# lightonai/next-plaid

Measured on AMD Instinct MI355X. Metric: queries/sec + p50 latency, k=10, 10M-doc x 300-tok x d128 PLAID index, 1/2/4/8 GPU, higher is better.
Workload: dtype f32 (split-bf16 hi/lo MFMA on the residual term of MaxSim, f32-class accuracy)

## Files before the change

next-plaid_amd/csrc/np_kernels.h:

```cpp
#pragma once
#include <hip/hip_runtime.h>
#include <stdint.h>
#include "np_exact.h"

namespace np {

__device__ __forceinline__ int wave_max_nonneg(int v) {
  v = max(v, __builtin_amdgcn_update_dpp(0, v, 0x111, 0xf, 0xf, false));
  v = max(v, __builtin_amdgcn_update_dpp(0, v, 0x112, 0xf, 0xf, false));
  v = max(v, __builtin_amdgcn_update_dpp(0, v, 0x114, 0xf, 0xf, false));
  v = max(v, __builtin_amdgcn_update_dpp(0, v, 0x118, 0xf, 0xf, false));
  v = max(v, __builtin_amdgcn_update_dpp(0, v, 0x142, 0xa, 0xf, false));
  v = max(v, __builtin_amdgcn_update_dpp(0, v, 0x143, 0xc, 0xf, false));
  return __builtin_amdgcn_readlane(v, 63);
}
template <int G, int J>
__device__ __forceinline__ int group_lane(int v, int lane) {
  if constexpr (G == 2) return __builtin_amdgcn_mov_dpp(v, J == 0 ? 0xA0 : 0xF5, 0xf, 0xf, true);
  else if constexpr (G == 4) return __builtin_amdgcn_mov_dpp(v, J == 0 ? 0x00 : 0x55, 0xf, 0xf, true);
  else return __shfl(v, (lane & ~(G - 1)) + J);
}

struct Counters {
  unsigned long long n_cells, n_ivf_ids, n_candidates, n_cand_tokens, n_exact_docs, n_exact_tokens, n_cand_codes;
// ... 982 lines not shown
    const uint32_t total = s_items[1024];
    for (uint32_t it = (uint32_t)wave; it < total; it += 16) {
      int a = 0, z = m;
      while (z - a > 1) {
        const int mid = (a + z) >> 1;
        if (s_items[mid] <= it) a = mid;
        else z = mid;
      }
      const uint32_t off = (it - s_items[a]) << 9, ln = s_len[a];
      const uint32_t* src = ivf + s_start[a] + off;
      uint32_t d[8];
#pragma unroll
      for (int k = 0; k < 8; ++k) {
        const uint32_t j = k * 64 + lane;
        d[k] = (off + j < ln) ? src[j] : 0xFFFFFFFFu;
      }
#pragma unroll
      for (int k = 0; k < 8; ++k) {
        const uint32_t rel = d[k] - lo;
        if (d[k] != 0xFFFFFFFFu && rel < span) {
          const uint32_t bit = 1u << (d[k] & 31);
          if (subset_bits && !(subset_bits[d[k] >> 5] & bit)) continue;
          atomicOr(&s_bits[rel >> 5], bit);
        }
      }
    }
  }
  __syncthreads();
  uint32_t* bits = docbits + (int64_t)b * NW + w0;
  for (int ch = wave; ch < slice_chunks; ch += 16) {
    const int64_t gch = (int64_t)sl * slice_chunks + ch;
    if (gch >= nchunks) break;
    int cnt = 0;
#pragma unroll
    for (int k = 0; k < NP_CHUNK_WORDS / 64; ++k) {
      const int w = ch * NP_CHUNK_WORDS + k * 64 + lane;
      if (w < nw) {
        const uint32_t v = s_bits[w];
        bits[w] = v;
        cnt += __popc(v);
      }
    }
#pragma unroll
    for (int o = 32; o > 0; o >>= 1) cnt += __shfl_xor(cnt, o);
    if (lane == 0) chunk_counts[(int64_t)b * nchunks + gch] = cnt;
  }
  if (sl == 0) {
#pragma unroll
    for (int o = 32; o > 0; o >>= 1) ids += __shfl_xor(ids, o);
    if (lane == 0 && ids) atomicAdd(&ctr->n_ivf_ids, ids);
  }
}

__global__ void __launch_bounds__(256) count_chunks_kernel(const uint32_t* __restrict__ docbits, int64_t NW,
                                                           int nchunks, int32_t* __restrict__ chunk_counts) {
  __shared__ int s_cnt;
  const int b = blockIdx.y, ch = blockIdx.x;
  if (threadIdx.x == 0) s_cnt = 0;
  __syncthreads();
  const uint32_t* bits = docbits + (int64_t)b * NW;
  int c = 0;
  for (int k = 0; k < NP_CHUNK_WORDS / 256; ++k) {
    const int64_t w = (int64_t)ch * NP_CHUNK_WORDS + k * 256 + threadIdx.x;
    if (w < NW) c += __popc(bits[w]);
  }
#pragma unroll
  for (int o = 32; o > 0; o >>= 1) c += __shfl_xor(c, o);
  if ((threadIdx.x & 63) == 0) atomicAdd(&s_cnt, c);
  __syncthreads();
  if (threadIdx.x == 0) chunk_counts[(int64_t)b * nchunks + ch] = s_cnt;
}

struct RoundPlan {
  int32_t* n_cand;
  int64_t* cand_base;
  int32_t* round_of;
  int32_t* round_tab;
  int32_t* order;
};

__global__ void __launch_bounds__(256) plan_rounds_kernel(const int32_t* __restrict__ chunk_counts, int nchunks, int B,
                                                          int64_t pool, int max_rounds, RoundPlan rp, Counters* ctr,
                                                          const int32_t* __restrict__ n_direct = nullptr ) {
  __shared__ int s_n[256];
  const int tid = threadIdx.x, lane = tid & 63, wave = tid >> 6;
  for (int b = wave; b < B; b += 4) {
    int c = 0;
    if (n_direct) c = lane == 0 ? n_direct[b] : 0;
    else
    for (int j = lane; j < nchunks; j += 64) c += chunk_counts[(int64_t)b * nchunks + j];
#pragma unroll
    for (int o = 32; o > 0; o >>= 1) c += __shfl_xor(c, o);
    if (lane == 0) s_n[b] = c;
  }
  __syncthreads();
  if (tid == 0) {
    int64_t cur = 0;
    unsigned long long total = 0;
    int r = 0;
    for (int i = 0; i < 2 * max_rounds; ++i) rp.round_tab[i] = 0;
    rp.round_tab[0] = 0;
    for (int b = 0; b < B; ++b) {
      const int n = s_n[b];
      if (cur + n > pool && r + 1 < max_rounds) {
        rp.round_tab[2 * r + 1] = b;
        ++r;
        rp.round_tab[2 * r] = b;
        cur = 0;
      }
      rp.n_cand[b] = (cur + n > pool) ? (int)max((int64_t)0, pool - cur) : n;
      rp.cand_base[b] = cur;
      rp.round_of[b] = r;
      cur += rp.n_cand[b];
      total += (unsigned long long)rp.n_cand[b];
    }
    rp.round_tab[2 * r + 1] = B;
    rp.round_tab[2 * max_rounds] = r + 1;
    if (!n_direct) atomicAdd(&ctr->n_candidates, total);
    atomicMax(&ctr->n_rounds, (unsigned long long)(r + 1));
  }
  __syncthreads();
  for (int b = tid; b < B; b += 256) {
    const int r = rp.round_of[b], rb = rp.round_tab[2 * r], re = rp.round_tab[2 * r + 1];
    const int n = rp.n_cand[b];
    int rank = 0;
    for (int j = rb; j < re; ++j) {
      const int nj = rp.n_cand[j];
      rank += (nj > n || (nj == n && j < b)) ? 1 : 0;
    }
    rp.order[rb + rank] = b;
  }
}

template <class Steal>
__device__ __forceinline__ int xcd_next_query(int32_t* slots, int32_t* ticket, int x, int step, int B,
                                              const int32_t* order, int rb, int re, Steal&& steal) {
  if (step > B) return -3;
  int32_t* slot = slots + (int64_t)x * (B + 1) + step;
  int v = __hip_atomic_load(slot, __ATOMIC_RELAXED, __HIP_MEMORY_SCOPE_AGENT);
  if (v == -1 && atomicCAS(slot, -1, -2) == -1) {
    const int t = atomicAdd(ticket, 1) + 1;
    v = (t < re - rb) ? order[rb + t] : steal();
    __hip_atomic_store(slot, v, __ATOMIC_RELAXED, __HIP_MEMORY_SCOPE_AGENT);
    return v;
  }
  while (v == -1 || v == -2) {
    __builtin_amdgcn_s_sleep(4);
    v = __hip_atomic_load(slot, __ATOMIC_RELAXED, __HIP_MEMORY_SCOPE_AGENT);
  }
  return v;
}

__global__ void __launch_bounds__(256) compact_kernel(const uint32_t* __restrict__ docbits, int64_t NW, int nchunks,
                                                      const int32_t* __restrict__ chunk_counts,
                                                      uint32_t* __restrict__ cand, RoundPlan rp, int round,
                                                      const uint4* __restrict__ doc_meta, uint4* __restrict__ cand_meta) {
  __shared__ int s_wave[4];
  __shared__ int s_base;
  const int b = blockIdx.y, ch = blockIdx.x, tid = threadIdx.x, lane = tid & 63, wave = tid >> 6;
  if (rp.round_of[b] != round) return;
  const int32_t* cc = chunk_counts + (int64_t)b * nchunks;
  {
    int part = 0;
    for (int j = tid; j < ch; j += 256) part += cc[j];
#pragma unroll
    for (int o = 32; o > 0; o >>= 1) part += __shfl_xor(part, o);
    if (lane == 0) s_wave[wave] = part;
    __syncthreads();
    if (tid == 0) s_base = s_wave[0] + s_wave[1] + s_wave[2] + s_wave[3];
    __syncthreads();
  }
  const int base = s_base;
  __syncthreads();
  const uint32_t* bits = docbits + (int64_t)b * NW;
  const int64_t w0 = (int64_t)ch * NP_CHUNK_WORDS + tid * 4;
  uint32_t w[4];
  int cnt = 0;
#pragma unroll
  for (int k = 0; k < 4; ++k) {
    w[k] = (w0 + k < NW) ? bits[w0 + k] : 0u;
    cnt += __popc(w[k]);
  }
  int incl = cnt;
#pragma unroll
  for (int o = 1; o < 64; o <<= 1) {
    int v = __shfl_up(incl, o);
    if (lane >= o) incl += v;
  }
  if (lane == 63) s_wave[wave] = incl;
  __syncthreads();
  int woff = 0;
  for (int k = 0; k < wave; ++k) woff += s_wave[k];
  int pos = base + woff + incl - cnt;
  const int limit = rp.n_cand[b];
  uint32_t* out = cand ? cand + rp.cand_base[b] : nullptr;
  uint4* outm = cand_meta + rp.cand_base[b];
#pragma unroll
  for (int k = 0; k < 4; ++k) {
    uint32_t m = w[k];
    while (m) {
      const int bit = __ffs(m) - 1;
      m &= m - 1;
      const uint32_t d = (uint32_t)((w0 + k) * 32 + bit);
      if (pos < limit) {
        if (doc_meta) outm[pos] = doc_meta[d];
        if (out) out[pos] = d;
      }
      ++pos;
    }
  }
}

#define NP_UB_BINS 2048
#define NP_GAIN_RANGE NP_IVF_SPLIT_RANGE
// ... 1324 lines not shown
      const uint32_t sum_lo = (uint32_t)max(slo, 0);
      if (valid && jl == 0) {
        U[pbase + i] = (uint16_t)sum;
        if (hb) atomicAdd(&s_hist[min(sum_lo >> hshift, (uint32_t)(NP_UB_BINS - 1))], 1u);
      }
      __builtin_amdgcn_wave_barrier();
    }
    __syncthreads();
    if (hb)
      for (int i = tid; i < NP_UB_BINS; i += 256) {
        const uint32_t v = s_hist[i];
        if (v) atomicAdd(&hb[i], v);
      }
  }
#pragma unroll
  for (int o = 32; o > 0; o >>= 1) {
    toks += __shfl_xor(toks, o);
    ucnt += __shfl_xor(ucnt, o);
    ndoc += __shfl_xor(ndoc, o);
  }
  __shared__ unsigned long long s_cnt[3];
  __syncthreads();
  if (tid == 0) s_cnt[0] = s_cnt[1] = s_cnt[2] = 0;
  __syncthreads();
  if (lane == 0 && toks) {
    atomicAdd(&s_cnt[0], toks);
    atomicAdd(&s_cnt[1], ucnt);
    atomicAdd(&s_cnt[2], ndoc);
  }
  __syncthreads();
  if (tid == 0 && s_cnt[0] && ctr) {
    if (count_tokens) {
      atomicAdd(&ctr->n_cand_tokens, s_cnt[0]);
      atomicAdd(&ctr->n_cand_dcodes, s_cnt[1]);
    } else {
      atomicAdd(&ctr->n_level2, s_cnt[2]);
    }
    atomicAdd(&ctr->n_cand_codes, s_cnt[1]);
  }
}

__global__ void __launch_bounds__(256) ub_thr_kernel(const uint32_t* __restrict__ hist, int hshift, int slack, int n_sel,
                                                     const int32_t* __restrict__ n_cand, RoundPlan rp, int round,
                                                     const uint32_t* __restrict__ qflag, uint32_t* __restrict__ thr) {
  __shared__ uint32_t s_part[256];
  constexpr int BPT = NP_UB_BINS / 256;
  const int b = blockIdx.x, tid = threadIdx.x;
  if (rp.round_of[b] != round) return;
  if (qflag[b] != 0 || n_cand[b] <= n_sel) {
    if (tid == 0) thr[b] = 0;
    return;
  }
  const uint32_t* hb = hist + (int64_t)b * NP_UB_BINS;
  const int top = (255 - tid) * BPT;
  uint32_t mine = 0;
#pragma unroll
  for (int k4 = 0; k4 < BPT / 4; ++k4) {
    const uint4 v = *reinterpret_cast<const uint4*>(hb + top + 4 * k4);
    mine += v.x + v.y + v.z + v.w;
  }
  s_part[tid] = mine;
  __syncthreads();
  if (tid == 0) {
    uint32_t cum = 0;
    int t = 0;
    for (; t < 255; ++t) {
      if (cum + s_part[t] >= (uint32_t)n_sel) break;
      cum += s_part[t];
    }
    int bin = (255 - t) * BPT + BPT - 1;
    for (; bin > (255 - t) * BPT; --bin) {
      if (cum + hb[bin] >= (uint32_t)n_sel) break;
      cum += hb[bin];
    }
    thr[b] = (uint32_t)max(0, bin - ((slack + (1 << hshift) - 1) >> hshift));
  }
}

struct CutP {
  const uint4* src;
  const int32_t* n_src_a;
  const int32_t* n_src_b;
  const uint16_t* U;
  const uint32_t* lo;
  const uint32_t* hi;
  int zero_mode;
  const uint4* all_src;
  const int32_t* n_all;
  uint4* dst;
  const int32_t* dst_begin;
  int32_t* n_dst;
  int hshift;
  Counters* ctr;
};

__global__ void __launch_bounds__(256) ub_cut_kernel(CutP p, RoundPlan rp, int round) {
  __shared__ int s_wcnt[4], s_base;
  __shared__ unsigned long long s_cnt[2];
  const int b = blockIdx.y, tid = threadIdx.x, lane = tid & 63, wave = tid >> 6;
  if (rp.round_of[b] != round) return;
  const uint32_t lo = p.lo[b], hi = p.hi ? p.hi[b] : 0xFFFFFFFFu;
  const bool all = lo == 0;
  if (all && p.zero_mode == 1) return;
  const uint4* src = all ? p.all_src : p.src;
  const int64_t n = all ? (int64_t)p.n_all[b] : (int64_t)p.n_src_a[b] + (p.n_src_b ? p.n_src_b[b] : 0);
  const int64_t pbase = rp.cand_base[b];
  const int64_t dbase = pbase + (p.dst_begin ? p.dst_begin[b] : 0);
  if (tid == 0) s_cnt[0] = s_cnt[1] = 0;
  unsigned long long toks = 0, ucnt = 0;
  constexpr int PT = 8;
  for (int64_t i0 = (int64_t)blockIdx.x * (256 * PT); i0 < n; i0 += (int64_t)gridDim.x * (256 * PT)) {
    bool keep[PT];
    unsigned long long bal[PT];
    int wtot = 0;
#pragma unroll
    for (int k = 0; k < PT; ++k) {
      const int64_t i = i0 + k * 256 + tid;
      bool kp = i < n;
      if (kp && !all) {
        const uint32_t bin = min((uint32_t)p.U[pbase + i] >> p.hshift, (uint32_t)(NP_UB_BINS - 1));
        kp = bin >= lo && bin < hi;
      }
      keep[k] = kp;
      bal[k] = __ballot(kp);
      wtot += (int)__popcll(bal[k]);
    }
    if (lane == 0) s_wcnt[wave] = wtot;
    __syncthreads();
    if (tid == 0) {
      const int tot = s_wcnt[0] + s_wcnt[1] + s_wcnt[2] + s_wcnt[3];
      s_base = tot ? atomicAdd(&p.n_dst[b], tot) : 0;
    }
    __syncthreads();
    int pos = s_base;
    for (int k = 0; k < wave; ++k) pos += s_wcnt[k];
#pragma unroll
    for (int k = 0; k < PT; ++k) {
      if (keep[k]) {
        const uint4 m = src[pbase + i0 + k * 256 + tid];
        p.dst[dbase + pos + (int)__popcll(bal[k] & ((1ull << lane) - 1ull))] = m;
        if (all) {
          toks += (unsigned long long)(m.w >> 8);
          ucnt += (unsigned long long)m.y;
        }
      }
      pos += (int)__popcll(bal[k]);
    }
    __syncthreads();
  }
  if (all && p.ctr) {
#pragma unroll
    for (int o = 32; o > 0; o >>= 1) {
      toks += __shfl_xor(toks, o);
      ucnt += __shfl_xor(ucnt, o);
    }
    if (lane == 0 && toks) {
      atomicAdd(&s_cnt[0], toks);
      atomicAdd(&s_cnt[1], ucnt);
    }
    __syncthreads();
    if (tid == 0 && s_cnt[0]) {
      atomicAdd(&p.ctr->n_cand_tokens, s_cnt[0]);
      atomicAdd(&p.ctr->n_cand_dcodes, s_cnt[1]);
      atomicAdd(&p.ctr->n_cand_codes, s_cnt[1]);
    }
  }
}

__global__ void __launch_bounds__(256) hot_prep_kernel(const uint8_t* __restrict__ QCU, int64_t K, int64_t KP, int RB,
                                                       uint8_t* __restrict__ cmaxu ,
                                                       uint32_t* __restrict__ chist ) {
  __shared__ uint32_t s_h[256];
  const int b = blockIdx.y, tid = threadIdx.x;
  s_h[tid] = 0;
  __syncthreads();
  for (int64_t c = (int64_t)blockIdx.x * 256 + tid; c < KP; c += (int64_t)gridDim.x * 256) {
    const uint4* row = reinterpret_cast<const uint4*>(QCU + ((int64_t)b * KP + c) * RB);
    uint32_t m = 0;
    for (int j = 0; j < RB / 16; ++j) {
      const uint4 v = row[j];
      const uint32_t w4[4] = {v.x, v.y, v.z, v.w};
#pragma unroll
      for (int e = 0; e < 4; ++e)
#pragma unroll
        for (int k = 0; k < 4; ++k) m = max(m, (w4[e] >> (8 * k)) & 0xFFu);
    }
    cmaxu[(int64_t)b * KP + c] = (uint8_t)m;
    if (c < K) atomicAdd(&s_h[m], 1u);
  }
  __syncthreads();
  if (s_h[tid]) atomicAdd(&chist[(int64_t)b * 256 + tid], s_h[tid]);
}

__global__ void __launch_bounds__(256) hot_lam_kernel(const uint32_t* __restrict__ chist, int64_t K, int hot_permille,
                                                      uint32_t* __restrict__ lam) {
  __shared__ uint32_t s_h[256];
  __shared__ uint32_t s_wsum[4];
  __shared__ int s_ok;
  const int b = blockIdx.x, v = threadIdx.x, lane = v & 63, wave = v >> 6;
  if (v == 0) s_ok = 0;
  uint32_t suf = chist[(int64_t)b * 256 + v];
#pragma unroll
  for (int o = 1; o < 64; o <<= 1) {
// ... 2350 lines not shown
```

next-plaid_amd/csrc/np_search.hip:

```cpp
#include "np_internal.h"
#include "np_kernels.h"

#include <algorithm>
#include <array>
#include <cmath>
#include <stdlib.h>
#include <string.h>
#include <type_traits>
#include <utility>

namespace np {

struct Workspace {
  DevBuf q, qoff, Qt, Qb, Qbl, QCT, gmax, tauq, cellbits, cells_tmp, cells, n_cells, docbits, chunk_counts, cand, cand_meta, approx, n_cand,
      cand_base, round_of, round_tab, QCU, qinv, qflag, ub, ub_hist, ub_thr, ub_cursor, q_order, xcd_slots, surv_meta, n_surv, n_list2, sel_keys, sel_doc, nsel, exact, out_ids, out_scores, out_keys, out_counts, ctr, subset,
      subset_bits, elig, misc, cut, cmaxu, chist, ub2, ub_hist2, ub_thr2, list_meta, n_l1, n_l2, qpad, planes, levels, hotbits,
      gain, gsmall, ghist, s0_meta, s0_u, gacc, gdeep,
      scan,
      filt, filt_csr;
  void* h_pin = nullptr;
  size_t h_pin_cap = 0;
  unsigned long long* h_gain = nullptr;
  uint64_t h_gain_key = 0;
  hipEvent_t done = nullptr;
// ... 1070 lines not shown
    hot_levels_kernel<<<dim3((unsigned)std::min<int64_t>(std::max<int64_t>((KP >> 5) / 256, 1), 16), B), 256, 0, st>>>(
        w.chist.as<uint32_t>(), ix->K, ix->tune.s4_hot, w.cmaxu.as<uint8_t>(), KP, ix->tune.s4_pexp, w.ub_thr2.as<uint32_t>() + B,
        w.levels.as<uint32_t>(), w.hotbits.as<uint32_t>(), p.s4_warm, w.ub_thr2.as<uint32_t>() + 2 * B,
        w.hotbits.as<uint32_t>() + (size_t)B * (KP / 32), ix->tune.s4_hot_auto ? w.n_cand.as<int32_t>() : nullptr,
        ix->tune.s4_hot_auto);
    const dim3 pg((unsigned)std::min<int64_t>((KP + 2047) / 2048, 64), B);
    with_int<32, 64>(p.RB, [&](auto RB) {
      hot_planes_kernel<RB><<<pg, 256, 0, st>>>(w.QCU.as<uint8_t>(), KP, w.cmaxu.as<uint8_t>(), w.ub_thr2.as<uint32_t>() + B,
                                                w.levels.as<uint32_t>(), w.planes.as<uint32_t>());
    });
  }
  return NP_OK;
}

int Pass::rounds(const RoundPlan& rp, const GainP& gp) const {
  SelectP sp;
  sp.approx = w.approx.as<float>();
  sp.cand = w.cand.as<uint32_t>();
  sp.cand_step = 1;
  sp.rp = rp;
  sp.n_cand = w.n_cand.as<int32_t>();
  sp.doc_begin = ix->doc_begin;
  sp.n_sel = cs->n_sel;
  sp.NSELP = cs->NSELP;
  sp.sel_keys = w.sel_keys.as<uint64_t>();
  sp.sel_doc = w.sel_doc.as<uint32_t>();
  sp.nsel_out = w.nsel.as<int32_t>();
  sp.ctr = nullptr;
  const size_t sel_lds = (size_t)cs->NSELP * 8;
  if (cs->n_sel > 0 && sel_lds > 48 * 1024)
    NP_HIP(hipFuncSetAttribute(reinterpret_cast<const void*>(&select_kernel),
                               hipFuncAttributeMaxDynamicSharedMemorySize, (int)sel_lds));
  for (int r = 0; r < (p.have_cands ? p.max_rounds : 0); ++r) NP_TRY(round(r, rp, gp, sp));
  return NP_OK;
}

int Pass::round(int r, const RoundPlan& rp, const GainP& gp, SelectP sp) const {
  const int B = p.B;
  if (p.gain_path)
    gain_emit_kernel<2><<<dim3((unsigned)ix->n_ranges, (unsigned)B), 256, 0, st>>>(gp, r);
  else
    compact_kernel<<<dim3(p.nchunks, B), 256, 0, st>>>(w.docbits.as<uint32_t>(), p.NW, p.nchunks, w.chunk_counts.as<int32_t>(),
                                                       (p.use_filter && !p.ids_only) ? nullptr : w.cand.as<uint32_t>(), rp, r,
                                                       p.ids_only ? nullptr : ix->d_doc_meta.get(), w.cand_meta.as<uint4>());
  if (cs->timed && r == 0) NP_HIP(hipEventRecord(cs->ctx->ev[3], st));
  const bool matvec = p.batched && !p.s1_split;
  if (p.use_filter) {
    NP_TRY(p.two_level ? two_level_cut(r, rp) : single_level_cut(r, rp));
    launch_approx(st, ix, w, d_qoff, B, p.LQP, w.surv_meta.as<uint4>(), w.n_surv.as<int32_t>(), rp, r, p.max_rounds, nullptr);
    sp.cand = reinterpret_cast<const uint32_t*>(w.surv_meta.p);
    sp.cand_step = 4;
    sp.n_cand = w.n_surv.as<int32_t>();
    sp.ctr = w.ctr.as<Counters>();
    if (matvec) {
      gcut_kernel<<<B, 1024, 0, st>>>(w.approx.as<float>(), w.surv_meta.as<uint4>(), w.n_surv.as<int32_t>(), rp, r, cs->n_sel,
                                      w.qinv.as<float>(), w.qflag.as<uint32_t>(), d_qoff, w.cand_meta.as<uint4>(),
                                      w.n_list2.as<int32_t>());
      launch_matvec(st, ix, w, d_q, d_qoff, B, w.cand_meta.as<uint4>(), w.n_list2.as<int32_t>(), rp, r);
      sp.cand = reinterpret_cast<const uint32_t*>(w.cand_meta.p);
      sp.n_cand = w.n_list2.as<int32_t>();
    }
  } else if (ix->T > 0) {
    if (matvec) {
      launch_matvec(st, ix, w, d_q, d_qoff, B, w.cand_meta.as<uint4>(), w.n_cand.as<int32_t>(), rp, r);
      count_work_kernel<<<dim3(32, (unsigned)B), 256, 0, st>>>(w.cand_meta.as<uint4>(), w.n_cand.as<int32_t>(), rp, r,
                                                               w.ctr.as<Counters>());
    } else {
      launch_approx(st, ix, w, d_qoff, B, p.LQP, w.cand_meta.as<uint4>(), w.n_cand.as<int32_t>(), rp, r, p.max_rounds,
                    w.ctr.as<Counters>());
    }
  }
  if (cs->timed && r == 0) NP_HIP(hipEventRecord(cs->ctx->ev[4], st));
  if (cs->n_sel > 0) {
    sp.round = r;
    select_kernel<<<B, 1024, (size_t)cs->NSELP * 8, st>>>(sp);
  }
  return NP_OK;
}

int Pass::single_level_cut(int r, const RoundPlan& rp) const {
  const int B = p.B;
  NP_TRY(ub_bounds(rp, r, p.max_rounds, slots((size_t)r * 3), cursor(0), w.cand_meta.as<uint4>(), nullptr, w.n_cand.as<int32_t>(),
                   w.n_cand.as<int32_t>(), w.ub.as<uint16_t>(), w.ub_hist.as<uint32_t>(), 1, 0, false));
  ub_thr_kernel<<<B, 256, 0, st>>>(w.ub_hist.as<uint32_t>(), p.hshift, p.slack, cs->n_sel, w.n_cand.as<int32_t>(), rp, r,
                                   w.qflag.as<uint32_t>(), w.ub_thr.as<uint32_t>());
  CutP cp{};
  cp.hshift = p.hshift;
  cp.all_src = w.cand_meta.as<uint4>();
  cp.n_all = w.n_cand.as<int32_t>();
  cp.src = w.cand_meta.as<uint4>();
  cp.n_src_a = w.n_cand.as<int32_t>();
  cp.U = w.ub.as<uint16_t>();
  cp.lo = w.ub_thr.as<uint32_t>();
  cp.zero_mode = 0;
  cp.dst = w.surv_meta.as<uint4>();
  cp.n_dst = w.n_surv.as<int32_t>();
  cp.ctr = w.ctr.as<Counters>();
  ub_cut_kernel<<<dim3(n_cut(), B), 256, 0, st>>>(cp, rp, r);
  return NP_OK;
}

int Pass::two_level_cut(int r, const RoundPlan& rp) const {
  const int B = p.B;
  const unsigned ncut = n_cut();
  auto ub = [&](int lvl, const int32_t* begin, const int32_t* count, int direct_wpq, bool floor_rows) {
    return ub_bounds(rp, r, p.max_rounds, slots((size_t)r * 3 + lvl), cursor(lvl), w.list_meta.as<uint4>(), begin, count,
                     w.n_cand.as<int32_t>(), w.ub2.as<uint16_t>(), w.ub_hist2.as<uint32_t>(), 0, direct_wpq, floor_rows);
  };
  CutP cp{};
  cp.hshift = p.hshift;
  cp.all_src = w.cand_meta.as<uint4>();
  cp.n_all = w.n_cand.as<int32_t>();
  if (cs->timed && r == 0) NP_HIP(hipEventRecord(cs->ctx->ev[8], st));
  NP_TRY(hot_level(r, rp));
  if (cs->timed && r == 0) {
    NP_HIP(hipEventRecord(cs->ctx->ev[9], st));
    cs->hot_timed = true;
  }
  ub_thr_kernel<<<B, 256, 0, st>>>(w.ub_hist.as<uint32_t>(), p.hshift, 0, cs->n_sel, w.n_cand.as<int32_t>(), rp, r,
                                   w.qflag.as<uint32_t>(), w.ub_thr.as<uint32_t>());
  cp.src = w.cand_meta.as<uint4>();
  cp.n_src_a = w.n_cand.as<int32_t>();
  cp.U = w.ub.as<uint16_t>();
  cp.lo = w.ub_thr.as<uint32_t>();
  cp.zero_mode = 1;
  cp.dst = w.list_meta.as<uint4>();
  cp.n_dst = w.n_l1.as<int32_t>();
  ub_cut_kernel<<<dim3(ncut, B), 256, 0, st>>>(cp, rp, r);
  NP_TRY(ub(1, nullptr, w.n_l1.as<int32_t>(), ix->tune.ub_direct, false));
  ub_thr_kernel<<<B, 256, 0, st>>>(w.ub_hist2.as<uint32_t>(), p.hshift, p.slack, cs->n_sel, w.n_cand.as<int32_t>(), rp, r,
                                   w.qflag.as<uint32_t>(), w.ub_thr2.as<uint32_t>());
  cp.lo = w.ub_thr2.as<uint32_t>();
  cp.hi = w.ub_thr.as<uint32_t>();
  cp.dst_begin = w.n_l1.as<int32_t>();
  cp.n_dst = w.n_l2.as<int32_t>();
  ub_cut_kernel<<<dim3(ncut, B), 256, 0, st>>>(cp, rp, r);
  NP_TRY(ub(2, w.n_l1.as<int32_t>(), w.n_l2.as<int32_t>(), 0, true));
  ub_thr_kernel<<<B, 256, 0, st>>>(w.ub_hist2.as<uint32_t>(), p.hshift, p.slack, cs->n_sel, w.n_cand.as<int32_t>(), rp, r,
                                   w.qflag.as<uint32_t>(), w.ub_thr2.as<uint32_t>());
  cp.src = w.list_meta.as<uint4>();
  cp.n_src_a = w.n_l1.as<int32_t>();
  cp.n_src_b = w.n_l2.as<int32_t>();
  cp.U = w.ub2.as<uint16_t>();
  cp.lo = w.ub_thr2.as<uint32_t>();
  cp.hi = nullptr;
  cp.zero_mode = 0;
  cp.dst = w.surv_meta.as<uint4>();
  cp.dst_begin = nullptr;
  cp.n_dst = w.n_surv.as<int32_t>();
  cp.ctr = w.ctr.as<Counters>();
  ub_cut_kernel<<<dim3(ncut, B), 256, 0, st>>>(cp, rp, r);
  return NP_OK;
}

int Pass::hot_level(int r, const RoundPlan& rp) const {
  const int B = p.B;
  const int64_t KP = p.KP;
  const int old_cap = ix->code_wide ? 64 : 128;
  const int plpd = (ix->ublock_stride > old_cap || ix->tune.s4_lpd == 4) ? 4 : 2;
  const unsigned pnbx = (unsigned)ix->tune.s4_pnbx;
  return with_codes(ix->code_wide, [&](auto ct) -> int {
    using CT = decltype(ct);
    if (!p.use_planes) {
      return with_rowb(p.RB, [&](auto RB) -> int {
        int32_t* sl = slots((size_t)r * 3);
        const size_t dyn = (size_t)(KP / 8);
        if (dyn > 16 * 1024)
          NP_HIP(hipFuncSetAttribute(reinterpret_cast<const void*>(&approx_hot_kernel<RB, CT>),
                                     hipFuncAttributeMaxDynamicSharedMemorySize, (int)dyn));
        approx_hot_kernel<RB, CT><<<8 * (unsigned)ix->tune.ub_nbx, 256, dyn, st>>>(
            w.QCU.as<uint8_t>(), ix->K, KP, w.cmaxu.as<uint8_t>(), w.ub_thr2.as<uint32_t>() + B, w.cand.as<uint32_t>(),
            w.cand_meta.as<uint4>(), ix->ublock_stride, (int64_t)ix->n_docs * ix->ublock_stride, w.n_cand.as<int32_t>(), rp, r,
            p.max_rounds, (const CT*)ix->d_ucodes.get(), w.qflag.as<uint32_t>(), d_qoff, cs->n_sel, w.ub.as<uint16_t>(),
            w.ub_hist.as<uint32_t>(), p.hshift, cursor(0), sl, sl + 8 * (B + 1), B, ix->tune.ub_steal, w.ctr.as<Counters>(),
            ix->tune.s4_probe, ix->tune.hot_static);
        return NP_OK;
      });
    }
    return with_int<32, 64>(p.RB, [&](auto RB) -> int {
      const int sb = ix->ublock_stride * (int)sizeof(CT);
      if constexpr (sizeof(CT) == 4) {
        if ((KP >> 3) >= 32 * 1024 && plpd == 4 && sb > 240 && sb <= 496)
          return hotp<RB, CT, 4, 1, 2, 0, 12>(r, rp, 32);
      }
      if (plpd == 2) {
        if (sb <= 240 && ix->tune.s4_qm) return hotp<RB, CT, 2, 2, 4, 1>(r, rp, pnbx);
        if (sb <= 240) return hotp<RB, CT, 2, 2, 4, 0>(r, rp, pnbx);
        return hotp<RB, CT, 2, 2, 2, 0>(r, rp, pnbx);
      }
      if (sb <= 240) return hotp<RB, CT, 4, 1, 4, 0>(r, rp, pnbx);
      if (sb <= 496) return hotp<RB, CT, 4, 1, 2, 0>(r, rp, pnbx);
      return hotp<RB, CT, 4, 1, 1, 0>(r, rp, pnbx);
    });
  });
}

template <int RB, class CT, int LPD, int PF, int DPI, int QM, int WPB>
int Pass::hotp(int r, const RoundPlan& rp, unsigned nbx) const {
  const int B = p.B;
  const int64_t KP = p.KP;
  int32_t* sl = slots((size_t)r * 3);
  const size_t bm = sizeof(CT) == 2 ? 0 : (size_t)(((KP >> 5) + 3) & ~(int64_t)3) * 4;
  const size_t rowb = (size_t)ix->ublock_stride * sizeof(CT) + 16;
  const int slack = (int)std::max<int64_t>(256, 1024 - (int64_t)DPI * (int64_t)rowb);
  const size_t dynp = bm + (size_t)WPB * ((64 / LPD) * rowb + (size_t)slack);
  if (dynp > 16 * 1024)
    NP_HIP(hipFuncSetAttribute(reinterpret_cast<const void*>(&approx_hotp_kernel<RB, CT, LPD, PF, DPI, QM, WPB>),
                               hipFuncAttributeMaxDynamicSharedMemorySize, (int)dynp));
  approx_hotp_kernel<RB, CT, LPD, PF, DPI, QM, WPB><<<8 * nbx, 64 * WPB, dynp, st>>>(
      w.planes.as<uint32_t>(), ix->K, KP, w.hotbits.as<uint32_t>(), w.ub_thr2.as<uint32_t>() + B, w.levels.as<uint32_t>(),
      w.cand.as<uint32_t>(), w.cand_meta.as<uint4>(), ix->ublock_stride, (int64_t)ix->n_docs * ix->ublock_stride,
      w.n_cand.as<int32_t>(), rp, r, p.max_rounds, (const CT*)ix->d_ucodes.get(), w.qflag.as<uint32_t>(), d_qoff, cs->n_sel,
      w.ub.as<uint16_t>(), w.ub_hist.as<uint32_t>(), p.hshift, sl, sl + 8 * (B + 1), B, w.ctr.as<Counters>(), slack,
      ix->tune.s4_probe, p.gain_path ? 1 : 0);
  return NP_OK;
}

static int phase_a_once(const DeviceIndex* ix, CallState* cs, const float* d_q, const int32_t* d_qoff,
                        const int32_t* h_qoff, const Subsets& sub, bool allow_grow) {
  Workspace& w = *cs->ctx->ws;
  hipStream_t st = cs->stream;
  PassPlan p;
  NP_TRY(plan_pass(ix, cs, h_qoff, sub, allow_grow, p));
  NP_TRY(reserve_pass(ix, cs, p, w));
  settle_zeroth_level(ix, w, cs, p);
  if (ix->ldim != ix->dim) {
    if (p.rows > 0)
// ... 1091 lines not shown
```

Before: 20630.

## Fuse threshold selection into ub_cut and stage round planning in LDS

```diff
diff --git a/next-plaid_amd/csrc/np_kernels.h b/next-plaid_amd/csrc/np_kernels.h
--- a/next-plaid_amd/csrc/np_kernels.h
+++ b/next-plaid_amd/csrc/np_kernels.h
@@ -1088,54 +1088,94 @@
 __global__ void __launch_bounds__(256) plan_rounds_kernel(const int32_t* __restrict__ chunk_counts, int nchunks, int B,
                                                           int64_t pool, int max_rounds, RoundPlan rp, Counters* ctr,
                                                           const int32_t* __restrict__ n_direct = nullptr ) {
-  __shared__ int s_n[256];
-  const int tid = threadIdx.x, lane = tid & 63, wave = tid >> 6;
-  for (int b = wave; b < B; b += 4) {
-    int c = 0;
-    if (n_direct) c = lane == 0 ? n_direct[b] : 0;
-    else
-    for (int j = lane; j < nchunks; j += 64) c += chunk_counts[(int64_t)b * nchunks + j];
-#pragma unroll
-    for (int o = 32; o > 0; o >>= 1) c += __shfl_xor(c, o);
-    if (lane == 0) s_n[b] = c;
+  __shared__ int s_n[256], s_nc[256], s_round[256], s_order[256], s_tab[2 * 256], s_nr;
+  __shared__ int64_t s_base[256];
+  const int tid = threadIdx.x;
+  if (n_direct) {
+    if (tid < B) s_n[tid] = n_direct[tid];
+  } else {
+    s_n[tid] = 0;
+    __syncthreads();
+    constexpr int DEEP = 8;
+    const uint32_t tot = (uint32_t)B * (uint32_t)nchunks, tot4 = tot / 4, nch = (uint32_t)nchunks;
+    const uint4* cc4 = reinterpret_cast<const uint4*>(chunk_counts);
+    for (uint32_t i0 = 0; i0 < tot4; i0 += 256 * DEEP) {
+      uint4 v[DEEP];
+#pragma unroll
+      for (int u = 0; u < DEEP; ++u) {
+        const uint32_t i = i0 + u * 256 + tid;
+        v[u] = i < tot4 ? cc4[i] : make_uint4(0, 0, 0, 0);
+      }
+#pragma unroll
+      for (int u = 0; u < DEEP; ++u) {
+        const uint32_t i = i0 + u * 256 + tid;
+        if (i >= tot4) continue;
+        const uint32_t b0 = 4 * i / nch, left = nch - (4 * i - b0 * nch);
+        const uint32_t w[4] = {v[u].x, v[u].y, v[u].z, v[u].w};
+        if (left >= 4) {
+          const int s = (int)(w[0] + w[1] + w[2] + w[3]);
+          if (s) atomicAdd(&s_n[b0], s);
+        } else {
+#pragma unroll
+          for (uint32_t e = 0; e < 4; ++e)
+            if (w[e]) atomicAdd(&s_n[b0 + (e >= left ? (e - left) / nch + 1 : 0)], (int)w[e]);
+        }
+      }
+    }
+    if ((uint32_t)tid < tot - 4 * tot4) {
+      const uint32_t i = 4 * tot4 + tid;
+      atomicAdd(&s_n[i / nch], chunk_counts[i]);
+    }
   }
   __syncthreads();
   if (tid == 0) {
     int64_t cur = 0;
     unsigned long long total = 0;
     int r = 0;
-    for (int i = 0; i < 2 * max_rounds; ++i) rp.round_tab[i] = 0;
-    rp.round_tab[0] = 0;
+    s_tab[0] = 0;
+#pragma unroll 8
     for (int b = 0; b < B; ++b) {
       const int n = s_n[b];
       if (cur + n > pool && r + 1 < max_rounds) {
-        rp.round_tab[2 * r + 1] = b;
+        s_tab[2 * r + 1] = b;
         ++r;
-        rp.round_tab[2 * r] = b;
+        s_tab[2 * r] = b;
         cur = 0;
       }
-      rp.n_cand[b] = (cur + n > pool) ? (int)max((int64_t)0, pool - cur) : n;
-      rp.cand_base[b] = cur;
-      rp.round_of[b] = r;
-      cur += rp.n_cand[b];
-      total += (unsigned long long)rp.n_cand[b];
-    }
-    rp.round_tab[2 * r + 1] = B;
-    rp.round_tab[2 * max_rounds] = r + 1;
+      const int nc = (cur + n > pool) ? (int)max((int64_t)0, pool - cur) : n;
+      s_nc[b] = nc;
+      s_base[b] = cur;
+      s_round[b] = r;
+      cur += nc;
+      total += (unsigned long long)nc;
+    }
+    s_tab[2 * r + 1] = B;
+    s_nr = r + 1;
     if (!n_direct) atomicAdd(&ctr->n_candidates, total);
     atomicMax(&ctr->n_rounds, (unsigned long long)(r + 1));
   }
   __syncthreads();
-  for (int b = tid; b < B; b += 256) {
-    const int r = rp.round_of[b], rb = rp.round_tab[2 * r], re = rp.round_tab[2 * r + 1];
-    const int n = rp.n_cand[b];
+  if (tid < B) {
+    const int b = tid, r = s_round[b], rb = s_tab[2 * r], re = s_tab[2 * r + 1];
+    const int n = s_nc[b];
     int rank = 0;
+#pragma unroll 8
     for (int j = rb; j < re; ++j) {
-      const int nj = rp.n_cand[j];
+      const int nj = s_nc[j];
       rank += (nj > n || (nj == n && j < b)) ? 1 : 0;
     }
-    rp.order[rb + rank] = b;
-  }
+    s_order[rb + rank] = b;
+  }
+  __syncthreads();
+  if (tid < B) {
+    rp.n_cand[tid] = s_nc[tid];
+    rp.cand_base[tid] = s_base[tid];
+    rp.round_of[tid] = s_round[tid];
+    rp.order[tid] = s_order[tid];
+  }
+  const int nr = s_nr;
+  for (int i = tid; i < 2 * max_rounds; i += 256) rp.round_tab[i] = i < 2 * nr ? s_tab[i] : 0;
+  if (tid == 0) rp.round_tab[2 * max_rounds] = nr;
 }
 
 template <class Steal>
@@ -2626,7 +2666,10 @@
   const int32_t* n_src_a;
   const int32_t* n_src_b;
   const uint16_t* U;
-  const uint32_t* lo;
+  const uint32_t* hist;
+  int slack, n_sel;
+  const uint32_t* qflag;
+  uint32_t* thr;
   const uint32_t* hi;
   int zero_mode;
   const uint4* all_src;
@@ -2638,22 +2681,79 @@
   Counters* ctr;
 };
 
+__device__ __forceinline__ void cut_bins(const uint32_t* __restrict__ hb, uint4& v0, uint4& v1) {
+  const int top = (255 - (int)threadIdx.x) * (NP_UB_BINS / 256);
+  v0 = *reinterpret_cast<const uint4*>(hb + top);
+  v1 = *reinterpret_cast<const uint4*>(hb + top + 4);
+}
+__device__ __forceinline__ uint32_t cut_threshold(const uint4 v0, const uint4 v1, int hshift, int slack, int n_sel) {
+  __shared__ uint32_t s_wsum[4], s_tstar, s_thr;
+  constexpr int BPT = NP_UB_BINS / 256;
+  static_assert(BPT == 8, "cut_threshold holds a partial's bins in two uint4");
+  const int tid = threadIdx.x, lane = tid & 63, wave = tid >> 6;
+  const int top = (255 - tid) * BPT;
+  const uint32_t mine = (v0.x + v0.y + v0.z + v0.w) + (v1.x + v1.y + v1.z + v1.w);
+  uint32_t incl = mine;
+#pragma unroll
+  for (int o = 1; o < 64; o <<= 1) {
+    const uint32_t up = __shfl_up(incl, o);
+    if (lane >= o) incl += up;
+  }
+  if (lane == 63) s_wsum[wave] = incl;
+  if (tid == 0) s_tstar = 255;
+  __syncthreads();
+  for (int k = 0; k < wave; ++k) incl += s_wsum[k];
+  const unsigned long long hit = __ballot(tid < 255 && incl >= (uint32_t)n_sel);
+  if (lane == 0 && hit) atomicMin(&s_tstar, (uint32_t)(wave * 64 + __ffsll((long long)hit) - 1));
+  __syncthreads();
+  if ((uint32_t)tid == s_tstar) {
+    const uint32_t h[BPT] = {v0.x, v0.y, v0.z, v0.w, v1.x, v1.y, v1.z, v1.w};
+    uint32_t cum = incl - mine;
+    int k = BPT - 1;
+#pragma unroll
+    for (int j = BPT - 1; j > 0; --j) {
+      if (k == j && cum + h[j] < (uint32_t)n_sel) {
+        cum += h[j];
+        k = j - 1;
+      }
+    }
+    s_thr = (uint32_t)max(0, top + k - ((slack + (1 << hshift) - 1) >> hshift));
+  }
+  __syncthreads();
+  return s_thr;
+}
+
 __global__ void __launch_bounds__(256) ub_cut_kernel(CutP p, RoundPlan rp, int round) {
   __shared__ int s_wcnt[4], s_base;
   __shared__ unsigned long long s_cnt[2];
   const int b = blockIdx.y, tid = threadIdx.x, lane = tid & 63, wave = tid >> 6;
   if (rp.round_of[b] != round) return;
-  const uint32_t lo = p.lo[b], hi = p.hi ? p.hi[b] : 0xFFFFFFFFu;
+  uint4 v0, v1;
+  cut_bins(p.hist + (int64_t)b * NP_UB_BINS, v0, v1);
+  const uint32_t flag = p.qflag[b], hi = p.hi ? p.hi[b] : 0xFFFFFFFFu;
+  const int n_all = p.n_all[b];
+  const int64_t n_src = (int64_t)p.n_src_a[b] + (p.n_src_b ? p.n_src_b[b] : 0);
+  const int64_t pbase = rp.cand_base[b];
+  const int64_t dbase = pbase + (p.dst_begin ? p.dst_begin[b] : 0);
+  constexpr int PT = 8;
+  const int64_t i00 = (int64_t)blockIdx.x * (256 * PT);
+  if (blockIdx.x > 0 && i00 >= max((int64_t)n_all, n_src)) return;
+  uint16_t u0[PT];
+#pragma unroll
+  for (int k = 0; k < PT; ++k) {
+    const int64_t i = i00 + k * 256 + tid;
+    u0[k] = i < n_src ? p.U[pbase + i] : (uint16_t)0;
+  }
+  uint32_t lo = cut_threshold(v0, v1, p.hshift, p.slack, p.n_sel);
+  if (flag != 0 || n_all <= p.n_sel) lo = 0;
+  if (blockIdx.x == 0 && tid == 0) p.thr[b] = lo;
   const bool all = lo == 0;
   if (all && p.zero_mode == 1) return;
   const uint4* src = all ? p.all_src : p.src;
-  const int64_t n = all ? (int64_t)p.n_all[b] : (int64_t)p.n_src_a[b] + (p.n_src_b ? p.n_src_b[b] : 0);
-  const int64_t pbase = rp.cand_base[b];
-  const int64_t dbase = pbase + (p.dst_begin ? p.dst_begin[b] : 0);
+  const int64_t n = all ? (int64_t)n_all : n_src;
   if (tid == 0) s_cnt[0] = s_cnt[1] = 0;
   unsigned long long toks = 0, ucnt = 0;
-  constexpr int PT = 8;
-  for (int64_t i0 = (int64_t)blockIdx.x * (256 * PT); i0 < n; i0 += (int64_t)gridDim.x * (256 * PT)) {
+  for (int64_t i0 = i00; i0 < n; i0 += (int64_t)gridDim.x * (256 * PT)) {
     bool keep[PT];
     unsigned long long bal[PT];
     int wtot = 0;
@@ -2662,7 +2762,8 @@
       const int64_t i = i0 + k * 256 + tid;
       bool kp = i < n;
       if (kp && !all) {
-        const uint32_t bin = min((uint32_t)p.U[pbase + i] >> p.hshift, (uint32_t)(NP_UB_BINS - 1));
+        const uint32_t u = i0 == i00 ? (uint32_t)u0[k] : (uint32_t)p.U[pbase + i];
+        const uint32_t bin = min(u >> p.hshift, (uint32_t)(NP_UB_BINS - 1));
         kp = bin >= lo && bin < hi;
       }
       keep[k] = kp;
diff --git a/next-plaid_amd/csrc/np_search.hip b/next-plaid_amd/csrc/np_search.hip
--- a/next-plaid_amd/csrc/np_search.hip
+++ b/next-plaid_amd/csrc/np_search.hip
@@ -1176,16 +1176,18 @@
   const int B = p.B;
   NP_TRY(ub_bounds(rp, r, p.max_rounds, slots((size_t)r * 3), cursor(0), w.cand_meta.as<uint4>(), nullptr, w.n_cand.as<int32_t>(),
                    w.n_cand.as<int32_t>(), w.ub.as<uint16_t>(), w.ub_hist.as<uint32_t>(), 1, 0, false));
-  ub_thr_kernel<<<B, 256, 0, st>>>(w.ub_hist.as<uint32_t>(), p.hshift, p.slack, cs->n_sel, w.n_cand.as<int32_t>(), rp, r,
-                                   w.qflag.as<uint32_t>(), w.ub_thr.as<uint32_t>());
   CutP cp{};
   cp.hshift = p.hshift;
+  cp.n_sel = cs->n_sel;
+  cp.qflag = w.qflag.as<uint32_t>();
   cp.all_src = w.cand_meta.as<uint4>();
   cp.n_all = w.n_cand.as<int32_t>();
   cp.src = w.cand_meta.as<uint4>();
   cp.n_src_a = w.n_cand.as<int32_t>();
   cp.U = w.ub.as<uint16_t>();
-  cp.lo = w.ub_thr.as<uint32_t>();
+  cp.hist = w.ub_hist.as<uint32_t>();
+  cp.slack = p.slack;
+  cp.thr = w.ub_thr.as<uint32_t>();
   cp.zero_mode = 0;
   cp.dst = w.surv_meta.as<uint4>();
   cp.n_dst = w.n_surv.as<int32_t>();
@@ -1203,6 +1205,8 @@
   };
   CutP cp{};
   cp.hshift = p.hshift;
+  cp.n_sel = cs->n_sel;
+  cp.qflag = w.qflag.as<uint32_t>();
   cp.all_src = w.cand_meta.as<uint4>();
   cp.n_all = w.n_cand.as<int32_t>();
   if (cs->timed && r == 0) NP_HIP(hipEventRecord(cs->ctx->ev[8], st));
@@ -1211,32 +1215,29 @@
     NP_HIP(hipEventRecord(cs->ctx->ev[9], st));
     cs->hot_timed = true;
   }
-  ub_thr_kernel<<<B, 256, 0, st>>>(w.ub_hist.as<uint32_t>(), p.hshift, 0, cs->n_sel, w.n_cand.as<int32_t>(), rp, r,
-                                   w.qflag.as<uint32_t>(), w.ub_thr.as<uint32_t>());
   cp.src = w.cand_meta.as<uint4>();
   cp.n_src_a = w.n_cand.as<int32_t>();
   cp.U = w.ub.as<uint16_t>();
-  cp.lo = w.ub_thr.as<uint32_t>();
+  cp.hist = w.ub_hist.as<uint32_t>();
+  cp.slack = 0;
+  cp.thr = w.ub_thr.as<uint32_t>();
   cp.zero_mode = 1;
   cp.dst = w.list_meta.as<uint4>();
   cp.n_dst = w.n_l1.as<int32_t>();
   ub_cut_kernel<<<dim3(ncut, B), 256, 0, st>>>(cp, rp, r);
   NP_TRY(ub(1, nullptr, w.n_l1.as<int32_t>(), ix->tune.ub_direct, false));
-  ub_thr_kernel<<<B, 256, 0, st>>>(w.ub_hist2.as<uint32_t>(), p.hshift, p.slack, cs->n_sel, w.n_cand.as<int32_t>(), rp, r,
-                                   w.qflag.as<uint32_t>(), w.ub_thr2.as<uint32_t>());
-  cp.lo = w.ub_thr2.as<uint32_t>();
+  cp.hist = w.ub_hist2.as<uint32_t>();
+  cp.slack = p.slack;
+  cp.thr = w.ub_thr2.as<uint32_t>();
   cp.hi = w.ub_thr.as<uint32_t>();
   cp.dst_begin = w.n_l1.as<int32_t>();
   cp.n_dst = w.n_l2.as<int32_t>();
   ub_cut_kernel<<<dim3(ncut, B), 256, 0, st>>>(cp, rp, r);
   NP_TRY(ub(2, w.n_l1.as<int32_t>(), w.n_l2.as<int32_t>(), 0, true));
-  ub_thr_kernel<<<B, 256, 0, st>>>(w.ub_hist2.as<uint32_t>(), p.hshift, p.slack, cs->n_sel, w.n_cand.as<int32_t>(), rp, r,
-                                   w.qflag.as<uint32_t>(), w.ub_thr2.as<uint32_t>());
   cp.src = w.list_meta.as<uint4>();
   cp.n_src_a = w.n_l1.as<int32_t>();
   cp.n_src_b = w.n_l2.as<int32_t>();
   cp.U = w.ub2.as<uint16_t>();
-  cp.lo = w.ub_thr2.as<uint32_t>();
   cp.hi = nullptr;
   cp.zero_mode = 0;
   cp.dst = w.surv_meta.as<uint4>();
```

After: 20790, median of 3. Within noise of the previous version (+0.8%).
